# ratt-ru/pfb-clean

Measured on AMD Instinct MI355X. Metric: PCG matvecs/sec (FFT-conv A^H A apply), 4k x 4k x 8-band cube, higher is better.
Workload: dtype f32; 1 GPU; 4096x4096x8-band cube PCG (hessian_psf + Tikhonov, M = x/sigmainv, tol=0, minit=maxit=20); nx_psf=8192, bands_per_gpu=8, parallelism=band-shard x1, allreduce_hook=False

## Files before the change

### include/pfb_hip.h

```cpp
#ifndef PFB_HIP_H
#define PFB_HIP_H

#include <stddef.h>
#include <stdint.h>

#ifdef __cplusplus
extern "C" {
#endif

#define PFB_ABI_VERSION 1

#define PFB_F32 0
#define PFB_F64 1

#define PFB_OK               0
#define PFB_ERR_INVALID     -1
#define PFB_ERR_UNSUPPORTED -2
#define PFB_ERR_HIP         -3
#define PFB_ERR_NONFINITE   -4
#define PFB_ERR_ALLOC       -5
#define PFB_ERR_COMM        -6

#define PFB_PCG_CONVERGED     0
#define PFB_PCG_MAXIT         1
// ... 49 lines not shown
int pfb_axpby(int dtype, double a, const void* x, double b, void* y, size_t n,
              void* stream);

typedef int (*pfb_allreduce_fn)(void* ctx, double* dev_buf, int count, void* stream);

typedef struct {
    int    status;
    int    iters;
    int    matvecs;
    int    backtracks;
    double eps;
    double rnorm;
} pfb_pcg_result;

size_t pfb_pcg_work_bytes(const pfb_conv_plan* plan, int nb);
int pfb_pcg_solve(pfb_conv_plan* plan, int band0, int nb,
                  const void* b, void* x, void* r_out,
                  const void* beam, double wsum, double sigmainv, double mdiv,
                  double tol, int maxit, int minit, int backtrack,
                  void* work, pfb_allreduce_fn allreduce, void* allreduce_ctx,
                  pfb_pcg_result* result, void* stream);

size_t pfb_pcg_bands_work_bytes(const pfb_conv_plan* plan, int nb);
int pfb_pcg_solve_bands(pfb_conv_plan* plan, int band0, int nb,
                        const void* b, void* x, void* r_out,
                        const void* beam, double wsum, double sigmainv, double mdiv,
                        double tol, int maxit, int minit, int backtrack,
                        void* work, pfb_pcg_result* results, void* stream);

int pfb_bandmix_dots(int dtype, const void* A, const void* c, int nband, size_t npix, double sigmainv,
// ... 250 lines not shown
```

### pfb_clean_amd/_lib.py

```python
import ctypes as C
import os

_HERE = os.path.dirname(os.path.abspath(__file__))
LIB_PATH = os.environ.get('PFB_HIP_LIB') or os.path.join(_HERE, 'libpfb_hip.so')

PFB_F32, PFB_F64 = 0, 1
PFB_OK = 0
ERRORS = {-1: 'invalid argument', -2: 'unsupported size/dtype', -3: 'HIP runtime error',
          -4: 'non-finite value', -5: 'device allocation failed', -6: 'band-shard exchange failed'}
PCG_STATUS = {0: 'converged', 1: 'maxit', 2: 'zero-residual', 3: 'breakdown'}
REDUCE_WS_DOUBLES = 8192


PFB_ERR_INVALID = -1
PFB_ERR_UNSUPPORTED = -2
PFB_ERR_ALLOC = -5
PFB_ERR_COMM = -6


class PfbHipError(RuntimeError):
    def __init__(self, code, msg):
        super().__init__(f"libpfb_hip: {ERRORS.get(code, code)}: {msg}")
        self.code = code

# ... 18 lines not shown
    'pfb_psfconv_plan_destroy': (_i, [_vp]),
    'pfb_psfconv_set_psfhat': (_i, [_vp, _vp, _vp]),
    'pfb_psfconv_apply': (_i, [_vp, _i, _i, _vp, _vp, _d, _d, _vp, _vp, _vp, _vp]),
    'pfb_psfconv_set_psf': (_i, [_vp, _vp, _vp, _vp]),
    'pfb_psfhat_regrid': (_i, [_i, _vp, _i, _i, _i, _i, _i, _i, _i, _vp, _vp]),
    'pfb_psfhat_from_psf': (_i, [_i, _vp, _i, _i, _i, _vp, _vp]),
    'pfb_psfconv_apply_dots': (_i, [_vp, _i, _i, _vp, _vp, _d, _d, _vp, _vp, _vp, _vp, _vp]),
    'pfb_psfconv_apply_dots_bands': (_i, [_vp, _i, _i, _vp, _vp, _d, _d, _vp, _vp, _vp, _vp, _vp]),
    'pfb_psfconv_plan_info': (_i, [_vp, C.POINTER(_i), C.POINTER(_i), C.POINTER(_sz)]),
    'pfb_psfconv_set_profiling': (_i, [_vp, _i]),
    'pfb_psfconv_get_profile': (_i, [_vp, C.POINTER(_d), C.POINTER(_i)]),
    'pfb_dot': (_i, [_i, _vp, _vp, _sz, _vp, _vp, _vp]),
    'pfb_norm_diff_sums': (_i, [_i, _vp, _vp, _sz, _vp, _vp, _vp]),
    'pfb_any_nonzero': (_i, [_i, _vp, _sz, _vp, _vp, _vp]),
    'pfb_axpby': (_i, [_i, _d, _vp, _d, _vp, _sz, _vp]),
    'pfb_pcg_work_bytes': (_sz, [_vp, _i]),
    'pfb_pcg_solve': (_i, [_vp, _i, _i, _vp, _vp, _vp, _vp, _d, _d, _d, _d, _i, _i, _i,
                           _vp, ALLREDUCE_FN, _vp, C.POINTER(PcgResult), _vp]),
    'pfb_pcg_bands_work_bytes': (_sz, [_vp, _i]),
    'pfb_pcg_solve_bands': (_i, [_vp, _i, _i, _vp, _vp, _vp, _vp, _d, _d, _d, _d, _i, _i, _i,
                                 _vp, C.POINTER(PcgResult), _vp]),
    'pfb_bandmix_dots': (_i, [_i, _vp, _vp, _i, _sz, _d, _vp, _vp, _vp, _vp, _vp, _vp]),
    'pfb_hessparam_work_bytes': (_sz, [_vp]),
    'pfb_hessparam_apply': (_i, [_vp, _vp, _vp, _vp, _d, _vp, _vp, _vp, _vp]),
    'pfb_hessparam_apply_dots': (_i, [_vp, _vp, _vp, _vp, _d, _vp, _vp, _vp, _vp, _vp, _vp, _vp]),
    'pfb_pcg_param_work_bytes': (_sz, [_vp, _i]),
    'pfb_pcg_solve_param': (_i, [_vp, _i, _vp, _vp, _vp, _vp, _vp, _vp, _d, _d, _d, _i, _i, _i,
                                 _vp, C.POINTER(PcgResult), _vp]),
    'pfb_comm_bind': (_i, [C.c_char_p]),
    'pfb_comm_unique_id': (_i, [_vp]),
# ... 114 lines not shown
```

### pfb_clean_amd/csrc/cgvec.hip

```cpp
#include "conv_plan.hpp"
#include "pcg_state.hpp"
#include "entry.hpp"
#include <chrono>
#include <unistd.h>
#include <cstring>
#include <cstdlib>
#include <utility>
#include <vector>

namespace pfb {

constexpr int RED_MAX_GRID = 1024;

static inline int red_grid(size_t nvec) {
    size_t g = (nvec + RED_BLOCK - 1) / RED_BLOCK;
    g = (g + 3) / 4;
    if (g < 1) g = 1;
    if (g > (size_t)RED_MAX_GRID) g = RED_MAX_GRID;
    return (int)g;
}

template <typename T, int V>
__global__ void __launch_bounds__(RED_BLOCK)
k_dot(const T* __restrict__ a, const T* __restrict__ b, size_t nvec, double* __restrict__ ws) {
// ... 140 lines not shown
    for (size_t i = (size_t)blockIdx.x * blockDim.x + threadIdx.x; i < nvec;
         i += (size_t)gridDim.x * blockDim.x) {
        Pack<T, V> pp = ld<T, V>(p, i), pr = ld<T, V>(r, i);
#pragma unroll
        for (int e = 0; e < V; ++e) {
            const T y = mdiv > T(0) ? pr.e[e] / mdiv : pr.e[e];
            const T v = beta * pp.e[e] - y;
            pp.e[e] = v;
            acc[0] += (v != T(0)) ? 1.0 : 0.0;
        }
        st<T, V>(p, i, pp);
    }
    emit_partials<1>(acc, ws);
}

template <typename T, int V, int U, bool XNT, bool REV>
__global__ void __launch_bounds__(RED_BLOCK)
k_pcg_update_dir(const T* x, const T* r, T* __restrict__ p, const T* __restrict__ Ap, T* xn, T* rn,
                 const double* __restrict__ S, T mdiv, size_t nvs, int gps, double* __restrict__ ws) {
    const int s = blockIdx.x / gps, g = blockIdx.x - s * gps;
    const double* Sb = S + (size_t)s * SB;
    { const size_t off = (size_t)s * nvs * V; x += off; r += off; p += off; Ap += off; xn += off; rn += off; }
    double acc[4] = {0.0, 0.0, 0.0, 0.0};
    if (sys_live(Sb)) {
        const T alpha = (T)Sb[S_ALPHA];
        const T beta = (T)Sb[S_BETA];
        const size_t stride = (size_t)gps * blockDim.x;
        for (size_t i0 = (size_t)g * blockDim.x + threadIdx.x; i0 < nvs; i0 += U * stride) {
            Pack<T, V> px[U], pr[U], pp[U], pa[U];
#pragma unroll
            for (int u = 0; u < U; ++u) {
                const size_t ii = i0 + u * stride;
                const size_t i = REV ? nvs - 1 - ii : ii;
                if (ii < nvs) {
                    px[u] = XNT ? ld_nt<T, V>(x, i) : ld<T, V>(x, i);
                    pr[u] = ld<T, V>(r, i); pp[u] = ld<T, V>(p, i); pa[u] = ld<T, V>(Ap, i);
                }
            }
#pragma unroll
            for (int u = 0; u < U; ++u) {
                const size_t ii = i0 + u * stride;
                const size_t i = REV ? nvs - 1 - ii : ii;
                if (ii >= nvs) break;
                Pack<T, V> ox, orr;
#pragma unroll
                for (int e = 0; e < V; ++e) {
                    const T xnew = px[u].e[e] + alpha * pp[u].e[e];
                    const T rnew = pr[u].e[e] + alpha * pa[u].e[e];
                    const T y = mdiv > T(0) ? rnew / mdiv : rnew;
                    ox.e[e] = xnew;
                    orr.e[e] = rnew;
                    const double d = (double)xnew - (double)px[u].e[e];
                    acc[0] += (double)rnew * (double)y;
                    acc[1] += d * d;
                    acc[2] += (double)xnew * (double)xnew;
                    const T pn = beta * pp[u].e[e] - y;
                    pp[u].e[e] = pn;
                    acc[3] += (pn != T(0)) ? 1.0 : 0.0;
                }
                if constexpr (XNT) st_nt<T, V>(xn, i, ox); else st<T, V>(xn, i, ox);
                st<T, V>(rn, i, orr);
                st<T, V>(p, i, pp[u]);
            }
        }
    } else if (xn != x) {
        for (size_t i = (size_t)g * blockDim.x + threadIdx.x; i < nvs; i += (size_t)gps * blockDim.x) {
            st<T, V>(xn, i, ld<T, V>(x, i));
            st<T, V>(rn, i, ld<T, V>(r, i));
        }
    }
    emit_partials<4>(acc, ws);
}

__global__ void k_set_alpha(double* S) { S[S_ALPHA] = S[S_RHO] / S[S_PAP]; S[S_NBT] = 0.0; }
__global__ void k_scale_alpha(double* S) { S[S_ALPHA] *= 0.75; }
__global__ void k_set_beta(double* S) { S[S_BETA] = S[S_RHON] / S[S_RHO]; }
__global__ void k_accept_rho(double* S) { S[S_RHO] = S[S_RHON]; }

__global__ void __launch_bounds__(256)
k_iter_sums(const double* __restrict__ cp, int bs, int qs, int bst, const double* __restrict__ ws, int gps,
            int have_upd, double* __restrict__ S, double mdiv, int predict, int logic) {
    __shared__ double vals[8];
    const int s = blockIdx.x, w = threadIdx.x >> 6, lane = threadIdx.x & 63;
    if (cp && w < 3) {
        const double* src = cp + (size_t)w * qs + (size_t)s * bst;
        double acc = 0.0;
        for (int k = lane; k < bs; k += 64) acc += src[k];
        acc = wave_sum(acc);
        if (lane == 0) vals[w] = acc;
    }
    if (have_upd && w < 4) {
        const double* src = ws + ((size_t)w * gridDim.x + s) * gps;
        double acc = 0.0;
        for (int g = lane; g < gps; g += 64) acc += src[g];
        acc = wave_sum(acc);
        if (lane == 0) vals[3 + w] = acc;
    }
    __syncthreads();
    double* Sb = S + (size_t)s * SB;
    if (threadIdx.x == 0 && sys_live(Sb)) {
        if (cp) { Sb[S_PAP] = vals[0]; Sb[S_RAP] = vals[1]; Sb[S_APAP] = vals[2]; }
        if (have_upd) { Sb[S_RHON] = vals[3]; Sb[S_NUM] = vals[4]; Sb[S_DEN] = vals[5]; Sb[S_ANY] = vals[6]; }
        if (logic) {
            if (have_upd) iter_end_dev(Sb);
            iter_begin_dev(Sb, mdiv, predict);
        }
    }
}
__global__ void __launch_bounds__(256)
k_iter_end(const double* __restrict__ ws, int gps, double* __restrict__ S) {
    __shared__ double vals[4];
    const int s = blockIdx.x, w = threadIdx.x >> 6, lane = threadIdx.x & 63;
    if (ws) {
        const double* src = ws + ((size_t)w * gridDim.x + s) * gps;
        double acc = 0.0;
        for (int g = lane; g < gps; g += 64) acc += src[g];
        acc = wave_sum(acc);
        if (lane == 0) vals[w] = acc;
        __syncthreads();
    }
    double* Sb = S + (size_t)s * SB;
    if (threadIdx.x == 0 && sys_live(Sb)) {
        if (ws) { Sb[S_RHON] = vals[0]; Sb[S_NUM] = vals[1]; Sb[S_DEN] = vals[2]; Sb[S_ANY] = vals[3]; }
        iter_end_dev(Sb);
    }
}
__global__ void k_iter_begin(double* S, double mdiv, int predict) { iter_begin_dev(S, mdiv, predict); }
__global__ void k_iter_end_begin(double* S, double mdiv, int predict) {
    iter_end_dev(S);
    iter_begin_dev(S, mdiv, predict);
}
__global__ void k_final_check(double* S, int nsys) {
    for (int s = threadIdx.x; s < nsys; s += blockDim.x) {
        double* Sb = S + (size_t)s * SB;
        if (Sb[S_ZERO] == 0.0 && Sb[S_DEAD] == 0.0 && Sb[S_ANY] == 0.0) {
            Sb[S_DEAD] = 1.0; Sb[S_K] -= 1.0; Sb[S_EPS] = Sb[S_EPSP];
        }
    }
}

#define PFB_LAUNCH_VEC(T, kern, n, ptrs, ...)                                              \
    do {                                                                                   \
        if (can_vec<T>(n, ptrs)) {                                                         \
            const size_t nvec = (n) / V16<T>::N;                                           \
            const int G = red_grid(nvec);                                                  \
// ... 53 lines not shown
    return (int)g;
}
static int update_grid(size_t nvs, int nsys) {
    int g = stream_grid(nvs);
    const int share = stream_grid((size_t)1 << 40) / nsys;
    if (g > share) g = share;
    if (g > RED_MAX_GRID / nsys) g = RED_MAX_GRID / nsys;
    return g < 1 ? 1 : g;
}
static int init_grid(size_t nvs, int nsys) {
    int g = red_grid(nvs);
    if (g > RED_MAX_GRID / nsys) g = RED_MAX_GRID / nsys;
    return g < 1 ? 1 : g;
}

struct PcgLayout {
    static constexpr size_t NONE = ~(size_t)0;
    size_t r, p, Ap, S, ws, xalt = NONE, ralt = NONE, tmp = NONE, mixp = NONE, total = 0;
    PcgLayout(const pfb_conv_plan* plan, int nb, int nsys, bool alternates, bool param) {
        auto take = [&](size_t bytes) { const size_t at = total; total += bytes; return at; };
        const size_t vb = vec_bytes(plan, nb);
        r = take(vb); p = take(vb); Ap = take(vb);
        S = take(((size_t)nsys * SB * sizeof(double) + 255) & ~(size_t)255);
        ws = take(sizeof(double) * 4 * (size_t)(nsys > RED_MAX_GRID ? nsys : RED_MAX_GRID));
        if (alternates) { xalt = take(vb); ralt = take(vb); }
        if (param) { const MixWork mw(plan); tmp = take(mw.total); mixp = tmp + mw.partials; }
    }
    template <typename U> U* at(void* work, size_t off) const { return off == NONE ? nullptr : (U*)((char*)work + off); }
};

struct PcgSync {
    pfb_allreduce_fn allreduce;
    void* actx;
    hipStream_t st;
    hipEvent_t ev = nullptr;
    double comm_timeout = 600.0;
    ~PcgSync() { if (ev) (void)hipEventDestroy(ev); }
    int open() {
        if (!allreduce) return PFB_OK;
        set_error("%s", "");
        if (const char* e = getenv("PFB_COMM_TIMEOUT_S")) { const double v = atof(e); if (v > 0) comm_timeout = v; }
// ... 100 lines not shown
};

template <typename T>
struct Pcg {
    pfb_conv_plan* plan;
    int nb;
    const T* b; T* x; T* r_out;
    double mdiv_d, tol;
    int maxit, minit;
    PcgSync sync;
    hipStream_t st;
    int nsys;
    size_t n, ns, nvs;
    bool vec;
    T *r, *p, *Ap, *xalt, *ralt;
    double *S, *ws;
    T mdiv;
    std::vector<double> h;
    PcgOp<T> A;

    explicit Pcg(const PcgSolve& q)
        : plan(q.plan), nb(q.nb), b((const T*)q.b), x((T*)q.x), r_out((T*)q.r_out), mdiv_d(q.mdiv), tol(q.tol),
          maxit(q.maxit), minit(q.minit), sync{q.allreduce, q.actx, q.st}, st(q.st), nsys(q.per_band ? q.nb : 1),
          mdiv((T)q.mdiv), h((size_t)nsys * SB) {
        n = (size_t)nb * plan->nx * plan->ny;
        ns = n / nsys;
        const PcgLayout lay(plan, nb, nsys, !q.per_band, q.L != nullptr);
        r = lay.at<T>(q.work, lay.r); p = lay.at<T>(q.work, lay.p); Ap = lay.at<T>(q.work, lay.Ap);
        S = lay.at<double>(q.work, lay.S); ws = lay.at<double>(q.work, lay.ws);
        xalt = lay.at<T>(q.work, lay.xalt); ralt = lay.at<T>(q.work, lay.ralt);
        A = {plan, q.band0, nb, nb / nsys, ns, q.per_band, (const T*)q.beam, q.wsum, q.sigmainv, (const T*)q.L,
             (const T*)q.LH, lay.at<T>(q.work, lay.tmp), lay.at<double>(q.work, lay.mixp), st};
        using PL = std::initializer_list<const void*>;
        vec = can_vec<T>(ns, PL{x, b, r, p, Ap});
        nvs = vec ? ns / V16<T>::N : ns;
    }

    int init() {
        int err;
        if ((err = sync.open()) != PFB_OK) return err;
        PFB_HIP_CHECK(hipMemsetAsync(S, 0, sizeof(double) * h.size(), st));
        if ((err = A.apply(x, r)) != PFB_OK) return err;
        const int gps = init_grid(nvs, nsys);
        if (vec)
            hipLaunchKernelGGL((k_pcg_init<T, V16<T>::N>), dim3(nsys * gps), dim3(RED_BLOCK), 0, st, r, b, p, mdiv, nvs,
                               gps, ws);
        else
            hipLaunchKernelGGL((k_pcg_init<T, 1>), dim3(nsys * gps), dim3(RED_BLOCK), 0, st, r, b, p, mdiv, nvs, gps, ws);
        const int hook = sync.allreduce ? 1 : 0;
        hipLaunchKernelGGL(k_init_state, dim3(nsys), dim3(RED_BLOCK), 0, st, (const double*)ws, gps, S, tol,
                           (double)minit, (double)maxit, 1, 1 - hook);
        if (hook) {
            if ((err = sync.reduce(S + S_RHON, 2)) != PFB_OK) return err;
            hipLaunchKernelGGL(k_init_state, dim3(nsys), dim3(RED_BLOCK), 0, st, (const double*)ws, gps, S, tol,
                               (double)minit, (double)maxit, 0, 1);
        }
// ... 15 lines not shown
            if (plan->pcg_pin) { PFB_HIP_CHECK(hipStreamSynchronize(st)); (void)hipHostFree(plan->pcg_pin); }
            plan->pcg_pin = nullptr;
            plan->pcg_pin_n = 0;
            PFB_HIP_CHECK(hipHostMalloc((void**)&plan->pcg_pin, sizeof(double) * 2 * nS, hipHostMallocDefault));
            plan->pcg_pin_n = nsys;
            for (int e = 0; e < 2; ++e)
                if (!plan->pcg_ev[e]) PFB_HIP_CHECK(hipEventCreateWithFlags(&plan->pcg_ev[e], hipEventDisableTiming));
        }
        const bool xnt = vec && n * sizeof(T) >= ((size_t)32 << 20);
        const double* seen = h.data();
        bool go = (1.0 > tol || 0 < minit) && 0 < maxit && any_live(seen);
        int khost = 0, slot = 0;
        bool pending_end = false, have_prev = false;
        int lo = 0, nl = nsys, gpl = update_grid(nvs, nsys);
        T *xc = x, *rc = r, *xn = xalt ? xalt : x, *rn = ralt ? ralt : r;
        auto narrow = [&](const double* hs) {
            int a = 0, z = nsys;
            while (a < z && !sys_live(hs + (size_t)a * SB)) ++a;
            while (z > a && !sys_live(hs + (size_t)(z - 1) * SB)) --z;
            if (z > a && (a != lo || z - a != nl)) { lo = a; nl = z - a; gpl = update_grid(nvs, nl); }
        };
        while (go) {
            const size_t off = (size_t)lo * ns;
            double* Sl = S + (size_t)lo * SB;
            typename PcgOp<T>::Partials c;
            if ((err = A.apply_partials(p, Ap, rc, lo, nl, &c)) != PFB_OK) return err;
            hipLaunchKernelGGL(k_iter_sums, dim3(nl), dim3(256), 0, st, c.cp, c.bs, c.qs, c.bst,
                               (const double*)ws, gpl, pending_end ? 1 : 0, Sl, mdiv_d, predict, hook ? 0 : 1);
            if (hook) {
                if ((err = sync.reduce(Sl + S_PAP, pending_end ? 7 : 4)) != PFB_OK) return err;
                if (pending_end) hipLaunchKernelGGL(k_iter_end_begin, dim3(1), dim3(1), 0, st, Sl, mdiv_d, predict);
                else hipLaunchKernelGGL(k_iter_begin, dim3(1), dim3(1), 0, st, Sl, mdiv_d, predict);
            }
            pending_end = false;
#define PFB_UPDATE(VV, XN)                                                                                     \
            hipLaunchKernelGGL((k_pcg_update_dir<T, VV, 2, XN, XN>), dim3(nl * gpl), dim3(RED_BLOCK), 0, st,   \
                               (const T*)xc + off, (const T*)rc + off, p + off, (const T*)Ap + off, xn + off,    \
                               rn + off, (const double*)Sl, mdiv, nvs, gpl, ws)
            if (xnt) PFB_UPDATE(V16<T>::N, true);
            else if (vec) PFB_UPDATE(V16<T>::N, false);
            else PFB_UPDATE(1, false);
#undef PFB_UPDATE
            std::swap(xc, xn);
            std::swap(rc, rn);
            if (khost + 1 < minit && khost + 1 < maxit) {
                pending_end = true;
            } else {
                if (hook) {
                    hipLaunchKernelGGL(k_iter_sums, dim3(nl), dim3(256), 0, st, (const double*)nullptr, 0, 0, 0,
                                       (const double*)ws, gpl, 1, Sl, mdiv_d, predict, 0);
                    if ((err = sync.reduce(Sl + S_RHON, 3)) != PFB_OK) return err;
                }
                hipLaunchKernelGGL(k_iter_end, dim3(nl), dim3(256), 0, st, hook ? nullptr : (const double*)ws, gpl, Sl);
            }
            PFB_HIP_CHECK(hipGetLastError());
            ++khost;
            if (khost < minit && khost < maxit) continue;
            if (lookahead && khost < maxit) {
                double* snap = plan->pcg_pin + (size_t)slot * nS;
                PFB_HIP_CHECK(hipMemcpyAsync(snap, S, sizeof(double) * nS, hipMemcpyDeviceToHost, st));
                PFB_HIP_CHECK(hipEventRecord(plan->pcg_ev[slot], st));
                if (have_prev) {
                    if ((err = sync.wait_event(plan->pcg_ev[slot ^ 1])) != PFB_OK) return err;
                    seen = plan->pcg_pin + (size_t)(slot ^ 1) * nS;
                    go = any_live(seen);
                    if (go) narrow(seen);
                }
                have_prev = true;
                slot ^= 1;
                continue;
            }
            if ((err = sync.fetch(h.data(), S, nS)) != PFB_OK) return err;
            seen = h.data();
            go = khost < maxit && any_live(seen);
            if (go) narrow(seen);
        }
        bool check = false;
        for (int s = 0; s < nsys; ++s) check |= seen[(size_t)s * SB + S_DEAD] == 0.0 && seen[(size_t)s * SB + S_ZERO] == 0.0;
        if (check) {
            if ((err = sync.reduce(S + S_ANY, 1)) != PFB_OK) return err;
            hipLaunchKernelGGL(k_final_check, dim3(1), dim3(64), 0, st, S, nsys);
            PFB_HIP_CHECK(hipGetLastError());
        }
        if (xc != x) PFB_HIP_CHECK(hipMemcpyAsync(x, xc, n * sizeof(T), hipMemcpyDeviceToDevice, st));
        if (r_out) PFB_HIP_CHECK(hipMemcpyAsync(r_out, rc, n * sizeof(T), hipMemcpyDeviceToDevice, st));
        return sync.fetch(h.data(), S, nS);
    }

    int run_exact() {
        using PL = std::initializer_list<const void*>;
        T *xcur = x, *rcur = r, *xnew = xalt, *rnew = ralt;
// ... 96 lines not shown
    return dtype == PFB_F32 ? nd_impl<float>(x, xp, n, out, ws, as_stream(stream))
                            : nd_impl<double>(x, xp, n, out, ws, as_stream(stream));
}

int pfb_any_nonzero(int dtype, const void* a, size_t n, double* out, double* ws, void* stream) {
    PFB_REQUIRE(a && out && ws, PFB_ERR_INVALID, "any_nonzero: null argument");
    return dtype == PFB_F32 ? any_impl<float>(a, n, out, ws, as_stream(stream))
                            : any_impl<double>(a, n, out, ws, as_stream(stream));
}

int pfb_axpby(int dtype, double a, const void* x, double b, void* y, size_t n, void* stream) {
    PFB_REQUIRE(x && y, PFB_ERR_INVALID, "axpby: null argument");
    return dtype == PFB_F32 ? axpby_impl<float>(a, x, b, y, n, as_stream(stream))
                            : axpby_impl<double>(a, x, b, y, n, as_stream(stream));
}
size_t pfb_pcg_work_bytes(const pfb_conv_plan* plan, int nb) {
    if (!plan || nb <= 0) return 0;
    return PcgLayout(plan, nb, 1, true, false).total;
}

int pfb_pcg_solve(pfb_conv_plan* plan, int band0, int nb, const void* b, void* x, void* r_out,
                  const void* beam, double wsum, double sigmainv, double mdiv, double tol,
                  int maxit, int minit, int backtrack, void* work, pfb_allreduce_fn allreduce,
                  void* allreduce_ctx, pfb_pcg_result* result, void* stream) {
    return pcg_checked("pcg_solve", {plan, band0, nb, false, b, x, r_out, beam, wsum, sigmainv, mdiv, tol, maxit, minit,
                                     backtrack, (size_t)4 << 20, work, allreduce, allreduce_ctx, nullptr, nullptr, result,
                                     as_stream(stream)});
}

size_t pfb_pcg_param_work_bytes(const pfb_conv_plan* plan, int nb) {
// ... 35 lines not shown
```

### pfb_clean_amd/csrc/conv_plan.hpp

```cpp
#pragma once
#include "common.hpp"
#include "fft_generic.hpp"

struct pfb_partial_layout {
    int slots, band_slots, q_stride, band_stride;
};

struct pfb_conv_plan {
    int nx, ny, P, Q, M;
    int nband, dtype;
    int VB, nvb;
    int fast;
    int long_lines;
    void* long_ws;
    size_t long_ws_bytes;
    pfb::FftFactors frow;
    pfb::FftFactors fcol;
    void* twP;
    void* twQ;
    void* psf_l;
    void* T;
    double* partials;
    size_t T_elems_per_band;
    size_t psf_elems_per_band;
    size_t workspace_bytes;
    int have_psf;
    int partials_per_band;
    pfb_partial_layout last;
    void* fast_tables;
    int prof_on, prof_n, prof_tick;
    hipEvent_t* prof_ev;
    double* pcg_pin;
    int pcg_pin_n;
    hipEvent_t pcg_ev[2];
};

namespace pfb {
inline size_t vec_bytes(const pfb_conv_plan* plan, int nb) {
    const size_t b = (size_t)nb * plan->nx * plan->ny * (plan->dtype == PFB_F32 ? 4 : 8);
    return (b + 255) & ~(size_t)255;
}
constexpr int PROF_MAX = 512;
inline void prof_mark(pfb_conv_plan* p, hipStream_t st, int k) {
    if (!p->prof_on) return;
    const bool sampled = (p->prof_tick % p->prof_on) == 0 && p->prof_n < PROF_MAX;
    if (sampled) (void)hipEventRecord(p->prof_ev[p->prof_n * 4 + k], st);
    if (k == 3) {
        if (sampled) p->prof_n++;
        p->prof_tick++;
// ... 25 lines not shown
```

### pfb_clean_amd/csrc/pcg_state.hpp

```cpp
#pragma once
#include "conv_plan.hpp"

namespace pfb {

enum { S_PAP = 0, S_RAP = 1, S_APAP = 2,
       S_ANY = 3,
       S_RHON = 4, S_NUM = 5, S_DEN = 6,
       S_RHO = 7, S_ALPHA = 8, S_BETA = 9, S_NBT = 10,
       S_DEAD = 11,
       S_K = 12, S_EPS = 13, S_EPSP = 14, S_NBTSUM = 15,
       S_STOP = 16,
       S_TOL = 17, S_MINIT = 18, S_MAXIT = 19,
       S_ZERO = 20,
       S_NSCALAR = 21 };
constexpr int SB = 32;
static_assert(S_NSCALAR <= SB, "state block too small");

__device__ __host__ __forceinline__ bool sys_live(const double* Sb) { return Sb[S_DEAD] == 0.0 && Sb[S_STOP] == 0.0; }

__device__ __forceinline__ void iter_begin_dev(double* S, double mdiv, int predict) {
    if (S[S_DEAD] != 0.0 || S[S_STOP] != 0.0) return;
    if (S[S_ANY] == 0.0) {
        S[S_DEAD] = 1.0;
        S[S_K] -= 1.0;
        S[S_EPS] = S[S_EPSP];
        return;
    }
    const double rho = S[S_RHO];
    double alpha = rho / S[S_PAP];
    int nbt = 0;
    if (predict == 1 || predict == 2) {
        const double d = mdiv > 0.0 ? mdiv : 1.0;
        const double s1 = S[S_RAP] / d, s2 = S[S_APAP] / d;
        while (rho + (2.0 * alpha * s1 + alpha * alpha * s2) > rho && nbt < 200) { alpha *= 0.75; ++nbt; }
    }
    S[S_ALPHA] = alpha;
    S[S_NBT] = (double)nbt;
    if (predict >= 2) {
        const double d = mdiv > 0.0 ? mdiv : 1.0;
        S[S_BETA] = (rho + (2.0 * alpha * S[S_RAP] + alpha * alpha * S[S_APAP]) / d) / rho;
    }
}
__device__ __forceinline__ void iter_end_dev(double* S) {
    if (S[S_DEAD] != 0.0 || S[S_STOP] != 0.0) return;
    S[S_RHO] = S[S_RHON];
    const double k = S[S_K] + 1.0;
    const double eps = sqrt(S[S_NUM] / (1e-12 + S[S_DEN]));
    S[S_K] = k;
    S[S_EPSP] = S[S_EPS];
    S[S_EPS] = eps;
    S[S_NBTSUM] += S[S_NBT];
    if (!((eps > S[S_TOL] || k < S[S_MINIT]) && k < S[S_MAXIT])) S[S_STOP] = 1.0;
}

constexpr int MIX_MAX_GRID = 1024;
int hessparam_apply_partials(pfb_conv_plan* plan, const void* L, const void* LH, const void* e, double sigmainv,
                             const void* x, void* out, const void* r, void* tmp, double* partials, int* grid,
                             hipStream_t st);
struct MixWork {
    size_t partials, total;
    explicit MixWork(const pfb_conv_plan* plan)
        : partials(vec_bytes(plan, plan->nband)), total(partials + sizeof(double) * 3 * MIX_MAX_GRID) {}
};

}
```

### pfb_clean_amd/operators/psf.py

```python
import ctypes as C
import threading

import torch

from .. import _lib, _dev
from .._plan import NativePlan, PlanCache, array_key


def _pow2ceil(n):
    p = 1
    while p < n:
        p *= 2
    return p


NX_FAST_MAX = 8192
NY_FAST_MAX = {torch.float32: 16384, torch.float64: 8192}
LINE_MAX = {torch.float32: 10240, torch.float64: 5120}
MIX_ALL = {
    'nx': {torch.float32: (96, 6144), torch.float64: (96, 6144)},
    'ny': {torch.float32: (160, 12288), torch.float64: (160, 6144)},
}
MIX_OFFERED = {
    'nx': {torch.float32: (), torch.float64: ()},
# ... 81 lines not shown
                    ph = ph2
                    cnx, cny, cpx, cpy = grid2[0], grid2[1], 2 * grid2[0], 2 * grid2[1]
        _lib.check(self._lib.pfb_psfconv_plan_create(cnx, cny, cpx, cpy, self.nband, self.code, C.byref(self._h)))
        try:
            if psf is None:
                _lib.check(self._lib.pfb_psfconv_set_psfhat(self._h, _dev.ptr(ph.contiguous()), _dev.stream()))
            else:
                _lib.check(self._lib.pfb_psfconv_set_psf(self._h, _dev.ptr(psf), _dev.ptr(psfhat_out), _dev.stream()))
        except Exception:
            self.close()
            raise
        torch.cuda.current_stream().synchronize()
        fast, vb, wsb = C.c_int(), C.c_int(), C.c_size_t()
        self._lib.pfb_psfconv_plan_info(self._h, C.byref(fast), C.byref(vb), C.byref(wsb))
        self.fast_path, self.vb, self.workspace_bytes = bool(fast.value), vb.value, wsb.value

    def _regrid(self, ph, grid2):
        nx2, ny2 = grid2
        cdt = ph.dtype
        need64 = 16 * self.nband * (self.nx_psf * self.nyo2 * 2 + 2 * nx2 * (ny2 + 1) * 2) + 8 * self.nband * (
            self.nx_psf * self.lastsize + 4 * nx2 * ny2) * 2
        try:
            free = torch.cuda.mem_get_info(ph.device)[0]
        except Exception:
            free = 0
        works = ((torch.complex128, 1), (cdt, self.code)) if need64 < 0.6 * free else ((cdt, self.code),)
        for work in works:
            src = ph.to(work[0]) if ph.dtype != work[0] else ph
            dst = torch.empty((self.nband, 2 * nx2, ny2 + 1), dtype=work[0], device=ph.device)
            rc = self._lib.pfb_psfhat_regrid(work[1], _dev.ptr(src), self.nband, self.nx, self.ny,
# ... 33 lines not shown
            cache[key] = (torch.zeros((nb,) + self.embed, dtype=self.rdtype, device=self.device),
                          torch.empty((nb,) + self.embed, dtype=self.rdtype, device=self.device))
        return cache[key]

    def _on_grid(self, fn_name, x, out, args):
        if self.embed is None:
            return self.run(fn_name, *args(x, out))
        with self.lock:
            xs, os_ = self._staging(x.shape[0], self._enter_stream())
            xs[:, :self.nx, :self.ny] = x
            self.run(fn_name, *args(xs, os_))
            out.copy_(os_[:, :self.nx, :self.ny])

    def _solve_work(self, kind, nb):
        cache = self.__dict__.setdefault('_work_cache', {})
        key = (kind, nb, _dev.stream(), threading.get_ident())
        if key not in cache:
            nbytes = getattr(self._lib, f'pfb_pcg_{kind}work_bytes')(self._h, nb)
            cache[key] = torch.empty(nbytes, dtype=torch.uint8, device=self.device)
        return cache[key]

    @classmethod
    def from_psf(cls, psf, nx, ny, want_psfhat=False, *, image=None):
        p = _dev.to_dev(psf)
        if p.ndim == 2:
            p = p[None]
        if p.ndim != 3 or p.dtype not in (torch.float32, torch.float64):
            raise ValueError("psf must be a real (nband, nx_psf, ny_psf) or (nx_psf, ny_psf) array")
        nband, nx_psf, ny_psf = (int(v) for v in p.shape)
        image = None if image is None or tuple(image) == (nx, ny) else tuple(int(v) for v in image)
        if _embed_grid(int(nx), int(ny), nx_psf, ny_psf, p.dtype) is not None:
# ... 98 lines not shown
```

Measured before the change: 443.1 cube-matvecs/s.

## Defer PCG solution updates into batched flushes over a ring of directions

During forced iterations (k < minit), the PCG direction update no longer reads or writes x. Each step's direction goes into a ring buffer of p slots, and its alpha is recorded in a device-side pending block. A flush kernel later applies up to `depth` x-updates in one pass and recovers the last two eps values for the convergence bookkeeping. This removes the per-iteration x read/write traffic, in exchange for extra workspace of `depth` vector-sized p slots, periodic flush passes that read every pending direction, and more intricate state handling.

```diff
diff --git a/include/pfb_hip.h b/include/pfb_hip.h
--- a/include/pfb_hip.h
+++ b/include/pfb_hip.h
@@ -87,6 +87,7 @@
 } pfb_pcg_result;
 
 size_t pfb_pcg_work_bytes(const pfb_conv_plan* plan, int nb);
+int pfb_pcg_set_defer(pfb_conv_plan* plan, int depth);
 int pfb_pcg_solve(pfb_conv_plan* plan, int band0, int nb,
                   const void* b, void* x, void* r_out,
                   const void* beam, double wsum, double sigmainv, double mdiv,
diff --git a/pfb_clean_amd/_lib.py b/pfb_clean_amd/_lib.py
--- a/pfb_clean_amd/_lib.py
+++ b/pfb_clean_amd/_lib.py
@@ -56,6 +56,7 @@
     'pfb_norm_diff_sums': (_i, [_i, _vp, _vp, _sz, _vp, _vp, _vp]),
     'pfb_any_nonzero': (_i, [_i, _vp, _sz, _vp, _vp, _vp]),
     'pfb_axpby': (_i, [_i, _d, _vp, _d, _vp, _sz, _vp]),
+    'pfb_pcg_set_defer': (_i, [_vp, _i]),
     'pfb_pcg_work_bytes': (_sz, [_vp, _i]),
     'pfb_pcg_solve': (_i, [_vp, _i, _i, _vp, _vp, _vp, _vp, _d, _d, _d, _d, _i, _i, _i,
                            _vp, ALLREDUCE_FN, _vp, C.POINTER(PcgResult), _vp]),
diff --git a/pfb_clean_amd/csrc/cgvec.hip b/pfb_clean_amd/csrc/cgvec.hip
--- a/pfb_clean_amd/csrc/cgvec.hip
+++ b/pfb_clean_amd/csrc/cgvec.hip
@@ -178,13 +178,23 @@
     emit_partials<1>(acc, ws);
 }
 
-template <typename T, int V, int U, bool XNT, bool REV>
+template <typename T>
+__device__ __forceinline__ T x_step(T x, T alpha, T p, double& num, double& den) {
+    T xnew;
+    if constexpr (sizeof(T) == 4) xnew = __builtin_fmaf(alpha, p, x); else xnew = __builtin_fma(alpha, p, x);
+    const double d = (double)xnew - (double)x;
+    num = __builtin_fma(d, d, num);
+    den = __builtin_fma((double)xnew, (double)xnew, den);
+    return xnew;
+}
+
+template <typename T, int V, int U, bool XNT, bool REV, bool LEAN>
 __global__ void __launch_bounds__(RED_BLOCK)
-k_pcg_update_dir(const T* x, const T* r, T* __restrict__ p, const T* __restrict__ Ap, T* xn, T* rn,
+k_pcg_update_dir(const T* x, const T* r, T* __restrict__ p, const T* __restrict__ Ap, T* xn, T* rn, T* __restrict__ pn,
                  const double* __restrict__ S, T mdiv, size_t nvs, int gps, double* __restrict__ ws) {
     const int s = blockIdx.x / gps, g = blockIdx.x - s * gps;
     const double* Sb = S + (size_t)s * SB;
-    { const size_t off = (size_t)s * nvs * V; x += off; r += off; p += off; Ap += off; xn += off; rn += off; }
+    { const size_t off = (size_t)s * nvs * V; x += off; r += off; p += off; Ap += off; xn += off; rn += off; pn += off; }
     double acc[4] = {0.0, 0.0, 0.0, 0.0};
     if (sys_live(Sb)) {
         const T alpha = (T)Sb[S_ALPHA];
@@ -197,7 +207,7 @@
                 const size_t ii = i0 + u * stride;
                 const size_t i = REV ? nvs - 1 - ii : ii;
                 if (ii < nvs) {
-                    px[u] = XNT ? ld_nt<T, V>(x, i) : ld<T, V>(x, i);
+                    if constexpr (!LEAN) px[u] = XNT ? ld_nt<T, V>(x, i) : ld<T, V>(x, i);
                     pr[u] = ld<T, V>(r, i); pp[u] = ld<T, V>(p, i); pa[u] = ld<T, V>(Ap, i);
                 }
             }
@@ -209,29 +219,69 @@
                 Pack<T, V> ox, orr;
 #pragma unroll
                 for (int e = 0; e < V; ++e) {
-                    const T xnew = px[u].e[e] + alpha * pp[u].e[e];
                     const T rnew = pr[u].e[e] + alpha * pa[u].e[e];
                     const T y = mdiv > T(0) ? rnew / mdiv : rnew;
-                    ox.e[e] = xnew;
                     orr.e[e] = rnew;
-                    const double d = (double)xnew - (double)px[u].e[e];
                     acc[0] += (double)rnew * (double)y;
-                    acc[1] += d * d;
-                    acc[2] += (double)xnew * (double)xnew;
-                    const T pn = beta * pp[u].e[e] - y;
-                    pp[u].e[e] = pn;
-                    acc[3] += (pn != T(0)) ? 1.0 : 0.0;
+                    if constexpr (!LEAN) ox.e[e] = x_step(px[u].e[e], alpha, pp[u].e[e], acc[1], acc[2]);
+                    const T pnew = beta * pp[u].e[e] - y;
+                    pp[u].e[e] = pnew;
+                    acc[3] += (pnew != T(0)) ? 1.0 : 0.0;
                 }
-                if constexpr (XNT) st_nt<T, V>(xn, i, ox); else st<T, V>(xn, i, ox);
+                if constexpr (!LEAN) { if constexpr (XNT) st_nt<T, V>(xn, i, ox); else st<T, V>(xn, i, ox); }
                 st<T, V>(rn, i, orr);
-                st<T, V>(p, i, pp[u]);
+                st<T, V>(LEAN ? pn : p, i, pp[u]);
             }
         }
-    } else if (xn != x) {
+    } else if (LEAN ? rn != r : xn != x) {
         for (size_t i = (size_t)g * blockDim.x + threadIdx.x; i < nvs; i += (size_t)gps * blockDim.x) {
-            st<T, V>(xn, i, ld<T, V>(x, i));
+            if constexpr (!LEAN) st<T, V>(xn, i, ld<T, V>(x, i));
             st<T, V>(rn, i, ld<T, V>(r, i));
         }
+    }
+    emit_partials<4>(acc, ws);
+}
+
+template <typename T, int V, int M, bool XNT, bool REV>
+__device__ __forceinline__ void flush_steps(T* x, const T* __restrict__ ring, size_t slot_elems,
+                                            const double* __restrict__ Pb, size_t nvs, int g, int gps, double (&acc)[4]) {
+    T alpha[M];
+    const T* pj[M];
+#pragma unroll
+    for (int j = 0; j < M; ++j) {
+        alpha[j] = (T)Pb[P_ALPHA + j];
+        pj[j] = ring + (size_t)Pb[P_SLOT + j] * slot_elems;
+    }
+    const size_t stride = (size_t)gps * blockDim.x;
+    for (size_t ii = (size_t)g * blockDim.x + threadIdx.x; ii < nvs; ii += stride) {
+        const size_t i = REV ? nvs - 1 - ii : ii;
+        Pack<T, V> px = XNT ? ld_nt<T, V>(x, i) : ld<T, V>(x, i), pp[M];
+#pragma unroll
+        for (int j = 0; j < M; ++j) pp[j] = XNT ? ld_nt<T, V>(pj[j], i) : ld<T, V>(pj[j], i);
+#pragma unroll
+        for (int j = 0; j < M; ++j) {
+            double unused[2] = {0.0, 0.0};
+            double* q = j == M - 1 ? acc + 2 : (j == M - 2 ? acc : unused);
+#pragma unroll
+            for (int e = 0; e < V; ++e) px.e[e] = x_step(px.e[e], alpha[j], pp[j].e[e], q[0], q[1]);
+        }
+        if constexpr (XNT) st_nt<T, V>(x, i, px); else st<T, V>(x, i, px);
+    }
+}
+template <typename T, int V, bool XNT, bool REV>
+__global__ void __launch_bounds__(RED_BLOCK)
+k_pcg_flush(T* x, const T* __restrict__ ring, size_t slot_elems, const double* __restrict__ Pd, size_t nvs, int gps,
+            double* __restrict__ ws) {
+    const int s = blockIdx.x / gps, g = blockIdx.x - s * gps;
+    const double* Pb = Pd + (size_t)s * PB;
+    { const size_t off = (size_t)s * nvs * V; x += off; ring += off; }
+    double acc[4] = {0.0, 0.0, 0.0, 0.0};
+    switch ((int)Pb[P_N]) {
+#define PFB_FLUSH(M) case M: flush_steps<T, V, M, XNT, REV>(x, ring, slot_elems, Pb, nvs, g, gps, acc); break;
+        PFB_FLUSH(1) PFB_FLUSH(2) PFB_FLUSH(3) PFB_FLUSH(4) PFB_FLUSH(5) PFB_FLUSH(6) PFB_FLUSH(7) PFB_FLUSH(8)
+        PFB_FLUSH(9) PFB_FLUSH(10) PFB_FLUSH(11) PFB_FLUSH(12) PFB_FLUSH(13) PFB_FLUSH(14) PFB_FLUSH(15) PFB_FLUSH(16)
+#undef PFB_FLUSH
+        default: break;
     }
     emit_partials<4>(acc, ws);
 }
@@ -243,7 +293,7 @@
 
 __global__ void __launch_bounds__(256)
 k_iter_sums(const double* __restrict__ cp, int bs, int qs, int bst, const double* __restrict__ ws, int gps,
-            int have_upd, double* __restrict__ S, double mdiv, int predict, int logic) {
+            int have_upd, double* __restrict__ S, double mdiv, int predict, int logic, double* __restrict__ Pd, int slot) {
     __shared__ double vals[8];
     const int s = blockIdx.x, w = threadIdx.x >> 6, lane = threadIdx.x & 63;
     if (cp && w < 3) {
@@ -266,8 +316,8 @@
         if (cp) { Sb[S_PAP] = vals[0]; Sb[S_RAP] = vals[1]; Sb[S_APAP] = vals[2]; }
         if (have_upd) { Sb[S_RHON] = vals[3]; Sb[S_NUM] = vals[4]; Sb[S_DEN] = vals[5]; Sb[S_ANY] = vals[6]; }
         if (logic) {
-            if (have_upd) iter_end_dev(Sb);
-            iter_begin_dev(Sb, mdiv, predict);
+            if (have_upd) iter_end_dev(Sb, Pd != nullptr);
+            iter_begin_dev(Sb, mdiv, predict, slot >= 0 ? Pd + (size_t)s * PB : nullptr, slot);
         }
     }
 }
@@ -286,13 +336,33 @@
     double* Sb = S + (size_t)s * SB;
     if (threadIdx.x == 0 && sys_live(Sb)) {
         if (ws) { Sb[S_RHON] = vals[0]; Sb[S_NUM] = vals[1]; Sb[S_DEN] = vals[2]; Sb[S_ANY] = vals[3]; }
-        iter_end_dev(Sb);
-    }
-}
-__global__ void k_iter_begin(double* S, double mdiv, int predict) { iter_begin_dev(S, mdiv, predict); }
-__global__ void k_iter_end_begin(double* S, double mdiv, int predict) {
-    iter_end_dev(S);
-    iter_begin_dev(S, mdiv, predict);
+        iter_end_dev(Sb, false);
+    }
+}
+__global__ void k_iter_begin(double* S, double mdiv, int predict, double* Pd, int slot) {
+    iter_begin_dev(S, mdiv, predict, slot >= 0 ? Pd : nullptr, slot);
+}
+__global__ void k_iter_end_begin(double* S, double mdiv, int predict, double* Pd, int slot) {
+    iter_end_dev(S, Pd != nullptr);
+    iter_begin_dev(S, mdiv, predict, slot >= 0 ? Pd : nullptr, slot);
+}
+__global__ void __launch_bounds__(256)
+k_flush_end(const double* __restrict__ ws, int gps, double* __restrict__ S, double* __restrict__ Pd, int sum, int logic) {
+    const int s = blockIdx.x, w = threadIdx.x >> 6, lane = threadIdx.x & 63;
+    __shared__ double vals[4];
+    double* Pb = Pd + (size_t)s * PB;
+    if (sum) {
+        const double* src = ws + ((size_t)w * gridDim.x + s) * gps;
+        double acc = 0.0;
+        for (int g = lane; g < gps; g += 64) acc += src[g];
+        acc = wave_sum(acc);
+        if (lane == 0) vals[w] = acc;
+        __syncthreads();
+    }
+    if (threadIdx.x == 0) {
+        if (sum) for (int q = 0; q < 4; ++q) Pb[P_SUMS + q] = vals[q];
+        if (logic) flush_end_dev(S + (size_t)s * SB, Pb);
+    }
 }
 __global__ void k_final_check(double* S, int nsys) {
     for (int s = threadIdx.x; s < nsys; s += blockDim.x) {
@@ -376,17 +446,33 @@
     return g < 1 ? 1 : g;
 }
 
+static int defer_depth(const pfb_conv_plan* plan, int nb) {
+    if (plan->pcg_defer) return plan->pcg_defer - 1;
+    static const size_t devmem = [] {
+        size_t fr = 0, tot = 0;
+        return hipMemGetInfo(&fr, &tot) == hipSuccess ? tot : (size_t)0;
+    }();
+    const size_t vb = vec_bytes(plan, nb);
+    if (vb < ((size_t)32 << 20)) return 0;
+    const size_t fit = devmem / 8 / vb;
+    const int d = fit > 8 ? 8 : (int)fit;
+    return d < 2 ? 0 : d;
+}
+
 struct PcgLayout {
     static constexpr size_t NONE = ~(size_t)0;
-    size_t r, p, Ap, S, ws, xalt = NONE, ralt = NONE, tmp = NONE, mixp = NONE, total = 0;
-    PcgLayout(const pfb_conv_plan* plan, int nb, int nsys, bool alternates, bool param) {
+    int depth;
+    size_t r, p, Ap, S, ws, xalt = NONE, ralt = NONE, tmp = NONE, mixp = NONE, pend = NONE, wsf = NONE, total = 0;
+    PcgLayout(const pfb_conv_plan* plan, int nb, int nsys, bool alternates, bool param) : depth(defer_depth(plan, nb)) {
         auto take = [&](size_t bytes) { const size_t at = total; total += bytes; return at; };
         const size_t vb = vec_bytes(plan, nb);
-        r = take(vb); p = take(vb); Ap = take(vb);
+        const size_t wsb = sizeof(double) * 4 * (size_t)(nsys > RED_MAX_GRID ? nsys : RED_MAX_GRID);
+        r = take(vb); p = take(vb * (size_t)(depth + 1)); Ap = take(vb);
         S = take(((size_t)nsys * SB * sizeof(double) + 255) & ~(size_t)255);
-        ws = take(sizeof(double) * 4 * (size_t)(nsys > RED_MAX_GRID ? nsys : RED_MAX_GRID));
+        ws = take(wsb);
         if (alternates) { xalt = take(vb); ralt = take(vb); }
         if (param) { const MixWork mw(plan); tmp = take(mw.total); mixp = tmp + mw.partials; }
+        if (depth > 0) { pend = take(((size_t)nsys * PB * sizeof(double) + 255) & ~(size_t)255); wsf = take(wsb); }
     }
     template <typename U> U* at(void* work, size_t off) const { return off == NONE ? nullptr : (U*)((char*)work + off); }
 };
@@ -517,7 +603,9 @@
     size_t n, ns, nvs;
     bool vec;
     T *r, *p, *Ap, *xalt, *ralt;
-    double *S, *ws;
+    double *S, *ws, *pend, *wsf;
+    int depth;
+    size_t slot_elems;
     T mdiv;
     std::vector<double> h;
     PcgOp<T> A;
@@ -532,17 +620,21 @@
         r = lay.at<T>(q.work, lay.r); p = lay.at<T>(q.work, lay.p); Ap = lay.at<T>(q.work, lay.Ap);
         S = lay.at<double>(q.work, lay.S); ws = lay.at<double>(q.work, lay.ws);
         xalt = lay.at<T>(q.work, lay.xalt); ralt = lay.at<T>(q.work, lay.ralt);
+        pend = lay.at<double>(q.work, lay.pend); wsf = lay.at<double>(q.work, lay.wsf);
+        slot_elems = vec_bytes(plan, nb) / sizeof(T);
         A = {plan, q.band0, nb, nb / nsys, ns, q.per_band, (const T*)q.beam, q.wsum, q.sigmainv, (const T*)q.L,
              (const T*)q.LH, lay.at<T>(q.work, lay.tmp), lay.at<double>(q.work, lay.mixp), st};
         using PL = std::initializer_list<const void*>;
         vec = can_vec<T>(ns, PL{x, b, r, p, Ap});
         nvs = vec ? ns / V16<T>::N : ns;
+        depth = vec ? lay.depth : 0;
     }
 
     int init() {
         int err;
         if ((err = sync.open()) != PFB_OK) return err;
         PFB_HIP_CHECK(hipMemsetAsync(S, 0, sizeof(double) * h.size(), st));
+        if (depth > 0) PFB_HIP_CHECK(hipMemsetAsync(pend, 0, sizeof(double) * (size_t)nsys * PB, st));
         if ((err = A.apply(x, r)) != PFB_OK) return err;
         const int gps = init_grid(nvs, nsys);
         if (vec)
@@ -588,6 +680,24 @@
         bool pending_end = false, have_prev = false;
         int lo = 0, nl = nsys, gpl = update_grid(nvs, nsys);
         T *xc = x, *rc = r, *xn = xalt ? xalt : x, *rn = ralt ? ralt : r;
+        T* pc = p;
+        int cur = 0, npend = 0;
+        auto deferred = [&](int k) { return depth > 0 && k + 1 < minit && k + 1 < maxit; };
+        auto flush = [&]() -> int {
+#define PFB_FLUSH(XN)                                                                                                \
+            hipLaunchKernelGGL((k_pcg_flush<T, V16<T>::N, XN, XN>), dim3(nsys * gpl), dim3(RED_BLOCK), 0, st, xc,   \
+                               (const T*)p, slot_elems, (const double*)pend, nvs, gpl, wsf)
+            if (xnt) PFB_FLUSH(true); else PFB_FLUSH(false);
+#undef PFB_FLUSH
+            hipLaunchKernelGGL(k_flush_end, dim3(nsys), dim3(256), 0, st, (const double*)wsf, gpl, S, pend, 1, hook ? 0 : 1);
+            if (hook) {
+                const int e = sync.reduce(pend + P_SUMS, 4);
+                if (e != PFB_OK) return e;
+                hipLaunchKernelGGL(k_flush_end, dim3(nsys), dim3(256), 0, st, (const double*)wsf, gpl, S, pend, 0, 1);
+            }
+            npend = 0;
+            return PFB_OK;
+        };
         auto narrow = [&](const double* hs) {
             int a = 0, z = nsys;
             while (a < z && !sys_live(hs + (size_t)a * SB)) ++a;
@@ -598,31 +708,40 @@
             const size_t off = (size_t)lo * ns;
             double* Sl = S + (size_t)lo * SB;
             typename PcgOp<T>::Partials c;
-            if ((err = A.apply_partials(p, Ap, rc, lo, nl, &c)) != PFB_OK) return err;
+            const bool lean = deferred(khost);
+            double* Pl = depth > 0 ? pend + (size_t)lo * PB : nullptr;
+            const int pslot = lean ? cur : -1;
+            if ((err = A.apply_partials(pc, Ap, rc, lo, nl, &c)) != PFB_OK) return err;
             hipLaunchKernelGGL(k_iter_sums, dim3(nl), dim3(256), 0, st, c.cp, c.bs, c.qs, c.bst,
-                               (const double*)ws, gpl, pending_end ? 1 : 0, Sl, mdiv_d, predict, hook ? 0 : 1);
+                               (const double*)ws, gpl, pending_end ? 1 : 0, Sl, mdiv_d, predict, hook ? 0 : 1, Pl, pslot);
             if (hook) {
                 if ((err = sync.reduce(Sl + S_PAP, pending_end ? 7 : 4)) != PFB_OK) return err;
-                if (pending_end) hipLaunchKernelGGL(k_iter_end_begin, dim3(1), dim3(1), 0, st, Sl, mdiv_d, predict);
-                else hipLaunchKernelGGL(k_iter_begin, dim3(1), dim3(1), 0, st, Sl, mdiv_d, predict);
+                if (pending_end) hipLaunchKernelGGL(k_iter_end_begin, dim3(1), dim3(1), 0, st, Sl, mdiv_d, predict, Pl, pslot);
+                else hipLaunchKernelGGL(k_iter_begin, dim3(1), dim3(1), 0, st, Sl, mdiv_d, predict, Pl, pslot);
             }
             pending_end = false;
-#define PFB_UPDATE(VV, XN)                                                                                     \
-            hipLaunchKernelGGL((k_pcg_update_dir<T, VV, 2, XN, XN>), dim3(nl * gpl), dim3(RED_BLOCK), 0, st,   \
-                               (const T*)xc + off, (const T*)rc + off, p + off, (const T*)Ap + off, xn + off,    \
-                               rn + off, (const double*)Sl, mdiv, nvs, gpl, ws)
-            if (xnt) PFB_UPDATE(V16<T>::N, true);
-            else if (vec) PFB_UPDATE(V16<T>::N, false);
-            else PFB_UPDATE(1, false);
+            const int nxt = cur == depth ? 0 : cur + 1;
+            T* pnx = p + (size_t)nxt * slot_elems;
+#define PFB_UPDATE(VV, XN, LEAN)                                                                                     \
+            hipLaunchKernelGGL((k_pcg_update_dir<T, VV, 2, XN, XN, LEAN>), dim3(nl * gpl), dim3(RED_BLOCK), 0, st,   \
+                               (const T*)xc + off, (const T*)rc + off, pc + off, (const T*)Ap + off, xn + off,        \
+                               rn + off, pnx + off, (const double*)Sl, mdiv, nvs, gpl, ws)
+            if (lean && xnt) PFB_UPDATE(V16<T>::N, true, true);
+            else if (lean) PFB_UPDATE(V16<T>::N, false, true);
+            else if (xnt) PFB_UPDATE(V16<T>::N, true, false);
+            else if (vec) PFB_UPDATE(V16<T>::N, false, false);
+            else PFB_UPDATE(1, false, false);
 #undef PFB_UPDATE
-            std::swap(xc, xn);
+            if (lean) { pc = pnx; cur = nxt; ++npend; }
+            else std::swap(xc, xn);
             std::swap(rc, rn);
             if (khost + 1 < minit && khost + 1 < maxit) {
                 pending_end = true;
+                if (npend > 0 && (npend == depth || !deferred(khost + 1)) && (err = flush()) != PFB_OK) return err;
             } else {
                 if (hook) {
                     hipLaunchKernelGGL(k_iter_sums, dim3(nl), dim3(256), 0, st, (const double*)nullptr, 0, 0, 0,
-                                       (const double*)ws, gpl, 1, Sl, mdiv_d, predict, 0);
+                                       (const double*)ws, gpl, 1, Sl, mdiv_d, predict, 0, (double*)nullptr, -1);
                     if ((err = sync.reduce(Sl + S_RHON, 3)) != PFB_OK) return err;
                 }
                 hipLaunchKernelGGL(k_iter_end, dim3(nl), dim3(256), 0, st, hook ? nullptr : (const double*)ws, gpl, Sl);
@@ -649,6 +768,7 @@
             go = khost < maxit && any_live(seen);
             if (go) narrow(seen);
         }
+        PFB_REQUIRE(npend == 0, PFB_ERR_INVALID, "pcg: %d deferred steps left pending at the end of the loop", npend);
         bool check = false;
         for (int s = 0; s < nsys; ++s) check |= seen[(size_t)s * SB + S_DEAD] == 0.0 && seen[(size_t)s * SB + S_ZERO] == 0.0;
         if (check) {
@@ -775,6 +895,14 @@
     return dtype == PFB_F32 ? axpby_impl<float>(a, x, b, y, n, as_stream(stream))
                             : axpby_impl<double>(a, x, b, y, n, as_stream(stream));
 }
+int pfb_pcg_set_defer(pfb_conv_plan* plan, int depth) {
+    static_assert(DEFER_MAX == 16, "k_pcg_flush's switch and the header state 16");
+    PFB_REQUIRE(plan, PFB_ERR_INVALID, "pcg_set_defer: null plan");
+    PFB_REQUIRE(depth >= -1 && depth <= DEFER_MAX, PFB_ERR_INVALID, "pcg_set_defer: depth %d outside -1..%d", depth, DEFER_MAX);
+    plan->pcg_defer = depth + 1;
+    return PFB_OK;
+}
+
 size_t pfb_pcg_work_bytes(const pfb_conv_plan* plan, int nb) {
     if (!plan || nb <= 0) return 0;
     return PcgLayout(plan, nb, 1, true, false).total;
diff --git a/pfb_clean_amd/csrc/conv_plan.hpp b/pfb_clean_amd/csrc/conv_plan.hpp
--- a/pfb_clean_amd/csrc/conv_plan.hpp
+++ b/pfb_clean_amd/csrc/conv_plan.hpp
@@ -33,6 +33,7 @@
     double* pcg_pin;
     int pcg_pin_n;
     hipEvent_t pcg_ev[2];
+    int pcg_defer;
 };
 
 namespace pfb {
diff --git a/pfb_clean_amd/csrc/pcg_state.hpp b/pfb_clean_amd/csrc/pcg_state.hpp
--- a/pfb_clean_amd/csrc/pcg_state.hpp
+++ b/pfb_clean_amd/csrc/pcg_state.hpp
@@ -16,14 +16,27 @@
 constexpr int SB = 32;
 static_assert(S_NSCALAR <= SB, "state block too small");
 
+constexpr int DEFER_MAX = 16;
+enum { P_N = 0,
+       P_OWED = 1,
+       P_SUMS = 2,
+       P_ALPHA = 6,
+       P_SLOT = P_ALPHA + DEFER_MAX,
+       P_NSCALAR = P_SLOT + DEFER_MAX };
+constexpr int PB = 40;
+static_assert(P_NSCALAR <= PB, "pending block too small");
+
+__device__ __forceinline__ double eps_of(double num, double den) { return sqrt(num / (1e-12 + den)); }
+
 __device__ __host__ __forceinline__ bool sys_live(const double* Sb) { return Sb[S_DEAD] == 0.0 && Sb[S_STOP] == 0.0; }
 
-__device__ __forceinline__ void iter_begin_dev(double* S, double mdiv, int predict) {
+__device__ __forceinline__ void iter_begin_dev(double* S, double mdiv, int predict, double* Pd, int slot) {
     if (S[S_DEAD] != 0.0 || S[S_STOP] != 0.0) return;
     if (S[S_ANY] == 0.0) {
         S[S_DEAD] = 1.0;
         S[S_K] -= 1.0;
-        S[S_EPS] = S[S_EPSP];
+        if (Pd && Pd[P_N] != 0.0) Pd[P_OWED] = 1.0;
+        else S[S_EPS] = S[S_EPSP];
         return;
     }
     const double rho = S[S_RHO];
@@ -40,17 +53,31 @@
         const double d = mdiv > 0.0 ? mdiv : 1.0;
         S[S_BETA] = (rho + (2.0 * alpha * S[S_RAP] + alpha * alpha * S[S_APAP]) / d) / rho;
     }
+    if (Pd) {
+        const int n = (int)Pd[P_N];
+        Pd[P_ALPHA + n] = alpha;
+        Pd[P_SLOT + n] = (double)slot;
+        Pd[P_N] = (double)(n + 1);
+    }
 }
-__device__ __forceinline__ void iter_end_dev(double* S) {
+__device__ __forceinline__ void iter_end_dev(double* S, bool deferred) {
     if (S[S_DEAD] != 0.0 || S[S_STOP] != 0.0) return;
     S[S_RHO] = S[S_RHON];
     const double k = S[S_K] + 1.0;
-    const double eps = sqrt(S[S_NUM] / (1e-12 + S[S_DEN]));
     S[S_K] = k;
+    S[S_NBTSUM] += S[S_NBT];
+    if (deferred) return;
+    const double eps = eps_of(S[S_NUM], S[S_DEN]);
     S[S_EPSP] = S[S_EPS];
     S[S_EPS] = eps;
-    S[S_NBTSUM] += S[S_NBT];
     if (!((eps > S[S_TOL] || k < S[S_MINIT]) && k < S[S_MAXIT])) S[S_STOP] = 1.0;
+}
+__device__ __forceinline__ void flush_end_dev(double* S, double* Pd) {
+    const int m = (int)Pd[P_N];
+    if (m >= 2) { S[S_EPSP] = S[S_EPS]; S[S_EPS] = eps_of(Pd[P_SUMS], Pd[P_SUMS + 1]); }
+    if (m >= 1) { S[S_EPSP] = S[S_EPS]; S[S_EPS] = eps_of(Pd[P_SUMS + 2], Pd[P_SUMS + 3]); }
+    if (Pd[P_OWED] != 0.0) { S[S_EPS] = S[S_EPSP]; Pd[P_OWED] = 0.0; }
+    Pd[P_N] = 0.0;
 }
 
 constexpr int MIX_MAX_GRID = 1024;
diff --git a/pfb_clean_amd/operators/psf.py b/pfb_clean_amd/operators/psf.py
--- a/pfb_clean_amd/operators/psf.py
+++ b/pfb_clean_amd/operators/psf.py
@@ -1,4 +1,5 @@
 import ctypes as C
+import os
 import threading
 
 import torch
@@ -119,6 +120,14 @@
         fast, vb, wsb = C.c_int(), C.c_int(), C.c_size_t()
         self._lib.pfb_psfconv_plan_info(self._h, C.byref(fast), C.byref(vb), C.byref(wsb))
         self.fast_path, self.vb, self.workspace_bytes = bool(fast.value), vb.value, wsb.value
+        self.pcg_defer = -1
+        if os.environ.get('PFB_PCG_DEFER', '') != '':
+            self.set_pcg_defer(int(os.environ['PFB_PCG_DEFER']))
+
+    def set_pcg_defer(self, depth):
+        with self.lock:
+            _lib.check(self._lib.pfb_pcg_set_defer(self._h, int(depth)))
+            self.pcg_defer = int(depth)
 
     def _regrid(self, ph, grid2):
         nx2, ny2 = grid2
@@ -182,7 +191,7 @@
 
     def _solve_work(self, kind, nb):
         cache = self.__dict__.setdefault('_work_cache', {})
-        key = (kind, nb, _dev.stream(), threading.get_ident())
+        key = (kind, nb, self.pcg_defer, _dev.stream(), threading.get_ident())
         if key not in cache:
             nbytes = getattr(self._lib, f'pfb_pcg_{kind}work_bytes')(self._h, nb)
             cache[key] = torch.empty(nbytes, dtype=torch.uint8, device=self.device)
```

Result: faster. 448.7 cube-matvecs/s, median of 6 (+1.3%).
